# imdea-software/legosnark

Hardware: AMD Instinct MI355X
Metric: alt_bn128 G1 MSM point-scalar pairs/s at n=2^20 (higher is better)
Workload: dtype u32 limbs (254-bit Montgomery integers)

## Files before the change

legosnark_amd/csrc/msm.hip:

```cpp
#include <hip/hip_runtime.h>
#include <stdint.h>
#include <stdio.h>
#include <stdlib.h>
#include <string.h>
#include <algorithm>
#include <type_traits>
#include <vector>

#include "curves.h"
#include "fp29x2l.h"
#include "fs29.h"
#include "glv.h"
#include "msm.h"
#include "msm_plan.h"

namespace lsa {

unsigned msm_window_bits(size_t n) {
    unsigned lg = 0;
    while ((size_t(1) << (lg + 1)) <= n) lg++;
    int c = (int)lg - 4;
    if (c < 8) c = 8;
    if (c > 16) c = 16;
    return (unsigned)c;
// ... 375 lines not shown
    for (uint32_t x = threadIdx.x; x < (Bc + 1) / 2; x += blockDim.x) cnt2[x] = 0;
    __syncthreads();
    const uint32_t t = xcd_tile(blockIdx.x, gridDim.x);
    const size_t lo = (size_t)t * tile;
    for (uint32_t il = threadIdx.x; il < tile; il += blockDim.x) {
        const size_t i = lo + il;
        if (i >= n) break;
        const uint32_t seg = segment_of(segs, (uint32_t)i);
        wide_digits(scalars[i], pl, seg * B, [&](unsigned, int32_t sd) {
            if (sd != 0) {
                const uint32_t b = cm.bin((uint32_t)(sd < 0 ? -sd : sd) - 1);
                atomicAdd(&cnt2[b >> 1], 1u << ((b & 1) * 16));
            }
        });
    }
    __syncthreads();
    uint16_t *th = tile_hist + (size_t)t * pitch;
    const uint16_t *c16 = reinterpret_cast<const uint16_t *>(cnt2);
    for (uint32_t x = threadIdx.x; x < Bc; x += blockDim.x) th[x] = c16[x];
}

template <int REC>
__global__ __launch_bounds__(1024) void k_scatter_wide(const Fr *__restrict__ scalars, size_t n, SegList segs, WidePlan pl, uint32_t B,
                                                       uint32_t Bc, uint32_t pitch, uint32_t tile, const uint32_t *__restrict__ hist_c,
                                                       uint32_t *__restrict__ offs, const uint32_t *__restrict__ tile_base,
                                                       void *__restrict__ out, uint32_t win_stride) {
    extern __shared__ __attribute__((aligned(16))) uint32_t base[];
    __shared__ uint32_t wsum[16];
    const uint32_t t = xcd_tile(blockIdx.x, gridDim.x);
    const uint32_t *tb = tile_base + (size_t)t * pitch;
    {
        const uint32_t per = (Bc + 1023) / 1024, b0 = threadIdx.x * per;
        uint32_t sum = 0;
        for (uint32_t q = 0; q < per; q++) if (b0 + q < Bc) sum += hist_c[b0 + q];
        uint32_t incl = sum;
#pragma unroll
        for (int d = 1; d < 64; d <<= 1) {
            const uint32_t u = __shfl_up(incl, d, 64);
            if ((int)(threadIdx.x & 63) >= d) incl += u;
        }
        if ((threadIdx.x & 63) == 63) wsum[threadIdx.x >> 6] = incl;
        __syncthreads();
        uint32_t run = incl - sum;
        for (uint32_t w = 0; w < (threadIdx.x >> 6); w++) run += wsum[w];
        for (uint32_t q = 0; q < per; q++) {
            const uint32_t b = b0 + q;
            if (b < Bc) {
                if (blockIdx.x == 0) offs[b] = run;
                base[b] = run + tb[b];
                run += hist_c[b];
            }
        }
    }
    __syncthreads();
    const size_t lo = (size_t)t * tile;
    for (uint32_t il = threadIdx.x; il < tile; il += 1024) {
        const size_t i = lo + il;
        if (i >= n) break;
        const uint32_t seg = segment_of(segs, (uint32_t)i);
        const uint32_t local = (uint32_t)i - segs.off[seg];
        wide_digits(scalars[i], pl, seg * B, [&](unsigned k, int32_t sd) {
            if (sd != 0) {
                const uint32_t b = (uint32_t)(sd < 0 ? -sd : sd) - 1;
                const uint32_t ent = (local + k * win_stride) | (sd < 0 ? 0x80000000u : 0u);
                if (REC == 1) ((uint64_t *)out)[atomicAdd(&base[b >> 7], 1u)] = ((uint64_t)(b & 127u) << 32) | ent;
                else if (REC == 2) ((uint32_t *)out)[atomicAdd(&base[b >> 6], 1u)] = (ent & 0x81ffffffu) | ((b & 63u) << 25);
                else ((uint32_t *)out)[atomicAdd(&base[b], 1u)] = ent;
            }
        });
    }
}

__device__ __forceinline__ uint32_t lds_inc_rank(uint32_t *counters, uint32_t idx) {
    const uint32_t first = (uint32_t)__builtin_amdgcn_readfirstlane((int)idx);
    const uint64_t active = __ballot(1), same = __ballot(idx == first);
    if (same == active) {
        const uint32_t rank = __builtin_amdgcn_mbcnt_hi((uint32_t)(active >> 32), __builtin_amdgcn_mbcnt_lo((uint32_t)active, 0u));
        uint32_t base = 0;
        if (rank == 0) base = atomicAdd(&counters[first], (uint32_t)__popcll(active));
        return (uint32_t)__builtin_amdgcn_readfirstlane((int)base) + rank;
    }
    return atomicAdd(&counters[idx], 1u);
}
#define PART_TILE 2048u
#define PART_SEGS 768u
#define PART_STAGE 28672u
__global__ __launch_bounds__(1024) void k_partition(const Fr *__restrict__ scalars, size_t n, SegList segs, WidePlan pl, uint32_t B, uint32_t Bc,
                                                    CoarseMap cm, uint32_t pitch, const uint16_t *__restrict__ tile_hist,
                                                    const uint32_t *__restrict__ hist_c, uint32_t *__restrict__ offs_c,
                                                    const uint32_t *__restrict__ tile_base, uint32_t *__restrict__ recs) {
    __builtin_amdgcn_s_setprio(3);
    extern __shared__ __attribute__((aligned(16))) uint32_t stage[];
    __shared__ uint32_t lstart[PART_SEGS + 1], lcur[PART_SEGS], gdst[PART_SEGS], wtot[2][PART_SEGS / 64];
    const uint32_t t = xcd_tile(blockIdx.x, gridDim.x);
    const unsigned lane = threadIdx.x & 63, wv = threadIdx.x >> 6;
    {
        uint32_t gv = 0, lv = 0;
        if (threadIdx.x < Bc) { gv = hist_c[threadIdx.x]; lv = tile_hist[(size_t)t * pitch + threadIdx.x]; }
        uint32_t gi = gv, li = lv;
#pragma unroll
        for (int d = 1; d < 64; d <<= 1) {
            const uint32_t a = __shfl_up(gi, d, 64), b = __shfl_up(li, d, 64);
            if ((int)lane >= d) { gi += a; li += b; }
        }
        if (wv < PART_SEGS / 64 && lane == 63) { wtot[0][wv] = gi; wtot[1][wv] = li; }
        __syncthreads();
        if (threadIdx.x < Bc) {
            uint32_t gex = gi - gv, lex = li - lv;
            for (unsigned w = 0; w < wv; w++) { gex += wtot[0][w]; lex += wtot[1][w]; }
            lstart[threadIdx.x] = lex;
            lcur[threadIdx.x] = lex;
            gdst[threadIdx.x] = gex + tile_base[(size_t)t * pitch + threadIdx.x];
            if (blockIdx.x == 0) offs_c[threadIdx.x] = gex;
            if (threadIdx.x == Bc - 1) lstart[Bc] = lex + lv;
        }
    }
    __syncthreads();
    const size_t lo = (size_t)t * PART_TILE;
    const uint32_t fine_bits = cm.sh_hi;
    const uint32_t tlow = t & ((1u << (16 - fine_bits)) - 1);
    for (uint32_t j = 0; j < PART_TILE / 1024; j++) {
        const uint32_t il = threadIdx.x + j * 1024;
        const size_t i = lo + il;
        if (i >= n) break;
        const uint32_t seg = segment_of(segs, (uint32_t)i);
        wide_digits(scalars[i], pl, seg * B, [&](unsigned k, int32_t sd) {
            if (sd != 0) {
                const uint32_t b = (uint32_t)(sd < 0 ? -sd : sd) - 1;
                const uint32_t pos = atomicAdd(&lcur[cm.bin(b)], 1u);
                stage[pos] = (tlow << (16 + fine_bits)) | (cm.fine(b) << 16) | (k << 12) | (sd < 0 ? 0x800u : 0u) | il;
            }
        });
    }
    __syncthreads();
    for (uint32_t sg = threadIdx.x >> 5; sg < Bc; sg += 32) {
        const uint32_t a = lstart[sg], e = lstart[sg + 1], g = gdst[sg];
        for (uint32_t x = a + (lane & 31); x < e; x += 32) recs[g + (x - a)] = stage[x];
    }
}

__global__ __launch_bounds__(1024) void k_fine_sort_part(const uint32_t *__restrict__ recs, const uint32_t *__restrict__ offs_c,
                                                         const uint32_t *__restrict__ hist_c, const uint32_t *__restrict__ tile_base,
                                                         uint32_t pitch, uint32_t T, CoarseMap cm, SegList segs, uint32_t win_stride, uint32_t stage_cap,
                                                         uint32_t *__restrict__ entries, uint32_t *__restrict__ hist, uint32_t *__restrict__ offs) {
    __builtin_amdgcn_s_setprio(3);
    extern __shared__ __attribute__((aligned(16))) uint32_t sm[];
    __shared__ uint32_t wsum[16];
    const uint32_t sg = blockIdx.x, lo = offs_c[sg], ns = hist_c[sg];
    const uint32_t fine_bits = cm.sh_hi, FM = 1u << fine_bits, fmask = FM - 1, tbits = 16 - fine_bits;
    const uint32_t F = 1u << cm.bits(sg), bucket0 = cm.first(sg);
    uint32_t *cnt = sm, *cur = sm + FM, *col = sm + 2 * FM, *stage = col + T + 1;
    const unsigned lane = threadIdx.x & 63, wv = threadIdx.x >> 6;
    for (uint32_t x = threadIdx.x; x < F; x += 1024) cnt[x] = 0;
    for (uint32_t x = threadIdx.x; x < T; x += 1024) col[x] = tile_base[(size_t)x * pitch + sg];
    if (threadIdx.x == 0) col[T] = ns;
    auto scan_counters = [&]() {
        const uint32_t per = (F + 1023) >> 10, f0 = threadIdx.x * per;
        uint32_t sum = 0;
        for (uint32_t q = 0; q < per; q++) if (f0 + q < F) sum += cnt[f0 + q];
        uint32_t incl = sum;
#pragma unroll
        for (int d = 1; d < 64; d <<= 1) {
            const uint32_t u = __shfl_up(incl, d, 64);
            if ((int)lane >= d) incl += u;
        }
        if (lane == 63) wsum[wv] = incl;
        __syncthreads();
        uint32_t run = incl - sum;
        for (unsigned w = 0; w < wv; w++) run += wsum[w];
        for (uint32_t q = 0; q < per; q++) {
            if (f0 + q >= F) break;
            const uint32_t c = cnt[f0 + q];
            cur[f0 + q] = run;
            hist[(size_t)bucket0 + f0 + q] = c;
            offs[(size_t)bucket0 + f0 + q] = lo + run;
            run += c;
        }
    };
    auto entry_of = [&](uint32_t r, uint32_t p2) {
        uint32_t a = 0, e = (T + (1u << tbits) - 1) >> tbits;
        while (e - a > 1) {
            const uint32_t m = (a + e) >> 1;
            if (col[m << tbits] <= p2) a = m; else e = m;
        }
        const uint32_t i = ((a << tbits) | (r >> (16 + fine_bits))) * PART_TILE + (r & 0x7ffu);
        const uint32_t local = i - segs.off[segment_of(segs, i)];
        return (local + ((r >> 12) & 15u) * win_stride) | ((r & 0x800u) << 20);
    };
    if (ns <= stage_cap) {
        constexpr uint32_t NR = PART_STAGE / 1024;
        uint32_t r[NR];
#pragma unroll
        for (uint32_t u = 0; u < NR; u++) { const uint32_t p2 = threadIdx.x + u * 1024; r[u] = p2 < ns ? recs[lo + p2] : 0u; }
        __syncthreads();
        uint16_t rk[NR];
#pragma unroll
        for (uint32_t u = 0; u < NR; u++) {
            rk[u] = 0;
            if (threadIdx.x + u * 1024 < ns) rk[u] = (uint16_t)atomicAdd(&cnt[(r[u] >> 16) & fmask], 1u);
        }
        __syncthreads();
        scan_counters();
        __syncthreads();
#pragma unroll
        for (uint32_t u = 0; u < NR; u++) {
            const uint32_t p2 = threadIdx.x + u * 1024;
            if (p2 < ns) stage[cur[(r[u] >> 16) & fmask] + rk[u]] = entry_of(r[u], p2);
        }
        __syncthreads();
        for (uint32_t x = threadIdx.x; x < ns; x += 1024) entries[lo + x] = stage[x];
        return;
    }
    __syncthreads();
    constexpr uint32_t UNR = 8;
    for (uint32_t p0 = threadIdx.x; p0 < ns; p0 += 1024 * UNR) {
        uint32_t r[UNR];
#pragma unroll
        for (uint32_t u = 0; u < UNR; u++) { const uint32_t p2 = p0 + u * 1024; r[u] = p2 < ns ? recs[lo + p2] : 0u; }
#pragma unroll
        for (uint32_t u = 0; u < UNR; u++) if (p0 + u * 1024 < ns) (void)lds_inc_rank(cnt, (r[u] >> 16) & fmask);
    }
    __syncthreads();
    scan_counters();
    __syncthreads();
    for (uint32_t p0 = threadIdx.x; p0 < ns; p0 += 1024 * UNR) {
        uint32_t r[UNR];
#pragma unroll
        for (uint32_t u = 0; u < UNR; u++) { const uint32_t p2 = p0 + u * 1024; r[u] = p2 < ns ? recs[lo + p2] : 0u; }
#pragma unroll
        for (uint32_t u = 0; u < UNR; u++) {
            const uint32_t p2 = p0 + u * 1024;
            if (p2 >= ns) break;
            entries[lo + lds_inc_rank(cur, (r[u] >> 16) & fmask)] = entry_of(r[u], p2);
        }
    }
}

template <class Rec>
struct RecOps;
template <>
struct RecOps<uint64_t> {
    static constexpr uint32_t NF = 128;
    static __device__ __forceinline__ uint32_t fine(uint64_t r) { return (uint32_t)(r >> 32); }
    static __device__ __forceinline__ uint32_t entry(uint64_t r) { return (uint32_t)r; }
};
template <>
struct RecOps<uint32_t> {
    static constexpr uint32_t NF = 64;
    static __device__ __forceinline__ uint32_t fine(uint32_t r) { return (r >> 25) & 63u; }
    static __device__ __forceinline__ uint32_t entry(uint32_t r) { return r & 0x81ffffffu; }
};
template <class Rec>
__global__ __launch_bounds__(1024) void k_fine_sort(const Rec *__restrict__ recs, const uint32_t *__restrict__ offs_c,
                                                    const uint32_t *__restrict__ hist_c, uint32_t *__restrict__ entries,
                                                    uint32_t *__restrict__ hist, uint32_t *__restrict__ offs) {
    using O = RecOps<Rec>;
    constexpr uint32_t NF = O::NF;
    __shared__ uint32_t cnt[NF], cur[NF];
    const uint32_t bin = blockIdx.x, lo = offs_c[bin], n = hist_c[bin];
    if (threadIdx.x < NF) cnt[threadIdx.x] = 0;
    __syncthreads();
    for (uint32_t j = threadIdx.x; j < n; j += 1024) atomicAdd(&cnt[O::fine(recs[lo + j])], 1u);
    __syncthreads();
    if (threadIdx.x < 64) {
        constexpr uint32_t PER = NF / 64;
        uint32_t c[PER], tot = 0;
#pragma unroll
        for (uint32_t q = 0; q < PER; q++) { c[q] = cnt[PER * threadIdx.x + q]; tot += c[q]; }
        uint32_t incl = tot;
#pragma unroll
        for (int d = 1; d < 64; d <<= 1) {
            uint32_t t = __shfl_up(incl, d, 64);
            if ((int)threadIdx.x >= d) incl += t;
        }
        uint32_t ex = incl - tot;
#pragma unroll
        for (uint32_t q = 0; q < PER; q++) {
            cur[PER * threadIdx.x + q] = ex;
            hist[(size_t)bin * NF + PER * threadIdx.x + q] = c[q];
            offs[(size_t)bin * NF + PER * threadIdx.x + q] = lo + ex;
            ex += c[q];
        }
    }
    __syncthreads();
    for (uint32_t j = threadIdx.x; j < n; j += 1024) {
        const Rec r = recs[lo + j];
        const uint32_t pos = atomicAdd(&cur[O::fine(r)], 1u);
        entries[lo + pos] = O::entry(r);
    }
}

#define SIZE_BINS 1025
__device__ __forceinline__ uint32_t size_bin(uint32_t cnt, uint32_t bin_shift) { return ((cnt - 1) >> bin_shift) + 1; }
template <class C>
__global__ __launch_bounds__(256) void k_size_hist(const uint32_t *__restrict__ hist, uint32_t nb, uint32_t thr, uint32_t *__restrict__ bin_count,
                                                   uint32_t group_size, uint32_t bin_shift) {
    bin_count += (group_size ? (blockIdx.x * 2048u) / group_size : 0u) * SIZE_BINS;
    __shared__ uint32_t lcnt[SIZE_BINS];
    for (uint32_t t = threadIdx.x; t < SIZE_BINS; t += 256) lcnt[t] = 0;
    __syncthreads();
    const uint32_t base = blockIdx.x * 2048 + threadIdx.x;
#pragma unroll
    for (int j = 0; j < 8; j++) {
        uint32_t g = base + j * 256;
        if (g < nb) { uint32_t cnt = hist[g]; if (cnt > 0 && cnt <= thr) atomicAdd(&lcnt[size_bin(cnt, bin_shift)], 1u); }
    }
    __syncthreads();
    for (uint32_t t = threadIdx.x; t < SIZE_BINS; t += 256) if (lcnt[t]) atomicAdd(&bin_count[t], lcnt[t]);
}
__global__ __launch_bounds__(256) void k_size_scan(const uint32_t *__restrict__ bin_count, uint32_t *__restrict__ bin_start, uint32_t ngroups) {
    __shared__ uint32_t lds[4];
    uint32_t carry = 0;
    for (uint32_t gidx = 0; gidx < ngroups; gidx++) {
        const uint32_t *bc = bin_count + gidx * SIZE_BINS;
        uint32_t *bs = bin_start + gidx * SIZE_BINS;
        uint32_t v[4], s = 0;
#pragma unroll
        for (int j = 0; j < 4; j++) {
            int bin = (int)SIZE_BINS - 1 - (int)(threadIdx.x * 4 + j);
            v[j] = (bin >= 1) ? bc[bin] : 0;
            s += v[j];
        }
        uint32_t tot;
        uint32_t run = carry + block_exclusive_scan_256(s, lds, &tot);
#pragma unroll
        for (int j = 0; j < 4; j++) {
            int bin = (int)SIZE_BINS - 1 - (int)(threadIdx.x * 4 + j);
            if (bin >= 1) bs[bin] = run;
            run += v[j];
        }
        carry += tot;
    }
    if (threadIdx.x == 0) bin_start[0] = carry;
}
template <class C>
__global__ __launch_bounds__(256) void k_size_scatter(const uint32_t *__restrict__ hist, uint32_t nb, uint32_t thr, const uint32_t *__restrict__ bin_start,
                                                      uint32_t *__restrict__ bin_cursor, uint32_t *__restrict__ perm,
                                                      uint32_t *__restrict__ heavy_list, uint32_t *__restrict__ heavy_count,
                                                      typename C::Acc *__restrict__ buckets, uint32_t group_size, uint32_t bin_shift,
                                                      uint32_t split) {
    const uint32_t goff = (group_size ? (blockIdx.x * 2048u) / group_size : 0u) * SIZE_BINS;
    bin_start += goff;
    bin_cursor += goff;
    __shared__ uint32_t lcnt[SIZE_BINS];
    for (uint32_t t = threadIdx.x; t < SIZE_BINS; t += 256) lcnt[t] = 0;
    __syncthreads();
    const uint32_t base = blockIdx.x * 2048 + threadIdx.x;
    uint32_t cnt[8], rank[8];
#pragma unroll
    for (int j = 0; j < 8; j++) {
        uint32_t g = base + j * 256;
        cnt[j] = 0; rank[j] = 0;
        if (g < nb) {
            cnt[j] = hist[g];
            if (cnt[j] == 0) { for (uint32_t h = 0; h < split; h++) buckets[(size_t)g * split + h] = C::inf(); }
            else if (cnt[j] > thr) heavy_list[atomicAdd(heavy_count, 1u)] = g;
            else rank[j] = atomicAdd(&lcnt[size_bin(cnt[j], bin_shift)], 1u);
        }
    }
    __syncthreads();
    for (uint32_t t = threadIdx.x; t < SIZE_BINS; t += 256) {
        uint32_t c = lcnt[t];
        lcnt[t] = c ? atomicAdd(&bin_cursor[t], c) : 0;
    }
    __syncthreads();
#pragma unroll
    for (int j = 0; j < 8; j++) {
        uint32_t g = base + j * 256;
        if (g < nb && cnt[j] > 0 && cnt[j] <= thr) {
            const uint32_t bin = size_bin(cnt[j], bin_shift);
            perm[bin_start[bin] + lcnt[bin] + rank[j]] = g;
        }
    }
}

template <class C, uint32_t ACC_SPLIT>
__device__ __forceinline__ void accumulate_body(const typename C::Base *__restrict__ bases, const uint32_t *__restrict__ entries,
                                                const uint32_t *__restrict__ offs, const uint32_t *__restrict__ hist,
                                                const uint32_t *__restrict__ perm, const uint32_t *__restrict__ nperm,
                                                typename C::Acc *__restrict__ buckets) {
    uint32_t t = blockIdx.x * blockDim.x + threadIdx.x;
    if (t >= *nperm * ACC_SPLIT) return;
    const uint32_t g = perm[t / ACC_SPLIT], part = t % ACC_SPLIT;
    const uint32_t cnt = hist[g];
    const uint32_t *e = entries + offs[g];
    typename C::Acc acc = C::inf();
    if (part < cnt) {
        uint32_t v = e[part];
        typename C::Base cur = bases[v & 0x3fffffffu];
        for (uint32_t j = part; j < cnt; j += ACC_SPLIT) {
            uint32_t vn = v;
            typename C::Base nxt = cur;
            if (j + ACC_SPLIT < cnt) { vn = e[j + ACC_SPLIT]; nxt = bases[vn & 0x3fffffffu]; }
            acc = C::madd(acc, cur, (v >> 31) != 0, ((v >> 30) & 1) != 0);
            v = vn;
            cur = nxt;
        }
    }
    buckets[(size_t)g * ACC_SPLIT + part] = acc;
}
template <class C, uint32_t ACC_SPLIT>
__global__ __launch_bounds__(256) void k_accumulate(const typename C::Base *__restrict__ bases, const uint32_t *__restrict__ entries,
                                                    const uint32_t *__restrict__ offs, const uint32_t *__restrict__ hist,
                                                    const uint32_t *__restrict__ perm, const uint32_t *__restrict__ nperm,
                                                    typename C::Acc *__restrict__ buckets) {
    accumulate_body<C, ACC_SPLIT>(bases, entries, offs, hist, perm, nperm, buckets);
}
__global__ __launch_bounds__(256) __attribute__((amdgpu_waves_per_eu(2, 2))) void k_accumulate_g2_occ2(
    const CurveG2::Base *__restrict__ bases, const uint32_t *__restrict__ entries, const uint32_t *__restrict__ offs,
    const uint32_t *__restrict__ hist, const uint32_t *__restrict__ perm, const uint32_t *__restrict__ nperm, CurveG2::Acc *__restrict__ buckets) {
    accumulate_body<CurveG2, 1u>(bases, entries, offs, hist, perm, nperm, buckets);
}

__global__ __launch_bounds__(256) void k_accumulate_g2_pair(const AffPackedG2 *__restrict__ bases, const uint32_t *__restrict__ entries,
                                                            const uint32_t *__restrict__ offs, const uint32_t *__restrict__ hist,
                                                            const uint32_t *__restrict__ perm, const uint32_t *__restrict__ nperm,
                                                            XYZZ29x2 *__restrict__ buckets) {
    const uint32_t t = blockIdx.x * blockDim.x + threadIdx.x, pr = t >> 1, part = t & 1;
    if (pr >= *nperm) return;
    const uint32_t g = perm[pr];
    const uint32_t cnt = hist[g];
    const uint32_t *e = entries + offs[g];
    struct Half { uint32_t x[8], y[8]; };
    auto fetch = [&](uint32_t v) {
        const AffPackedG2 &b = bases[v & 0x3fffffffu];
        Half h;
#pragma unroll
        for (int i = 0; i < 8; i++) { h.x[i] = b.w[part][i]; h.y[i] = b.w[2 + part][i]; }
        return h;
    };
    XyzzE<F29h> acc = XyzzE<F29h>::inf();
    uint32_t v = e[0];
    Half cur = fetch(v);
    for (uint32_t j = 0; j < cnt; j++) {
        uint32_t vn = v;
        Half nxt = cur;
        if (j + 1 < cnt) { vn = e[j + 1]; nxt = fetch(vn); }
        AffE<F29h> q = {{F29::unpack256(cur.x)}, {F29::unpack256(cur.y)}};
        if (!q.is_inf()) {
            if (v >> 31) q.y = sub_k<1>(F29h::zero(), q.y);
            acc = g2_madd(acc, q);
        }
        v = vn;
        cur = nxt;
    }
    F29 *o = reinterpret_cast<F29 *>(&buckets[g]);
    o[part] = acc.X.v;
    o[2 + part] = acc.Y.v;
    o[4 + part] = acc.ZZ.v;
    o[6 + part] = acc.ZZZ.v;
}

template <class A>
__device__ __forceinline__ A shfl_down_acc(const A &p, unsigned delta) {
    A r;
// ... 663 lines not shown
    typename C::Base *tbl = (typename C::Base *)d_table;
    hipLaunchKernelGGL((k_shift_window<C>), dim3((unsigned)((n + 255) / 256)), dim3(256), 0, st, tbl + (size_t)(k - 1) * n, (Jac<F> *)d_tmp, n, grid.pos[k] - grid.pos[k - 1]);
    return prepare_bases<F>((const Jac<F> *)d_tmp, tbl + (size_t)k * n, n, st);
}
template int precompute_window_step<Fq>(void *, size_t, void *, unsigned, hipStream_t);
template int precompute_window_step<Fq2>(void *, size_t, void *, unsigned, hipStream_t);
template int precompute_windows<Fq>(void *, size_t, hipStream_t);
template int precompute_windows<Fq2>(void *, size_t, hipStream_t);

unsigned msm_field_mults_per_pair(size_t n, size_t table_n) {
    if (table_n && n >= table_use_min()) return wide_plan(table_n, n, 1).nwin * 10;
    return 16 * 10 + 8;
}

template <class F>
static int msm_pipeline(const void *d_bases_v, size_t first, const Fr *d_scalars, const SegList &segs, Jac<F> *d_out, hipStream_t st,
                        size_t table_stride, bool reuse_sort = false, bool blocking = false) {
    using C = typename CurveOf<F>::type;
    using A = typename C::Acc;
    const typename C::Base *d_bases = (const typename C::Base *)d_bases_v + first;
    const uint32_t nseg = segs.nseg;
    const size_t n = segs.off[nseg];
    if (n >= (size_t(1) << 27)) { set_error("msm: n too large (%zu)", n); return LSA_ERR_INVALID; }
    const bool wide = table_stride != 0 && (nseg > 1 || n >= table_use_min());
    if (nseg > 1 && !wide) { set_error("msm: segmented calls need bases with pre-shifted copies"); return LSA_ERR_INVALID; }
    WidePlan pl = {};
    if (wide) {
        pl = wide_plan(table_stride, n, nseg);
        if ((uint64_t)table_stride * table_copies(table_stride) >= (1u << 30)) { set_error("msm: base table too large for 30-bit entries"); return LSA_ERR_INVALID; }
    }
    const bool glv = C::GLV && !wide;
    const unsigned c = wide ? pl.c : msm_window_bits(glv ? 2 * n : n);
    const unsigned nwin = wide ? pl.nwin : (glv ? (128 + c - 1) / c : num_windows(c));
    const size_t nv = glv ? 2 * n : n;
    const uint32_t B = 1u << (c - 1);
    const uint32_t nb = wide ? nseg * B : nwin * B;
    if (wide && (uint64_t)nseg * B > (1u << 21)) { set_error("msm: %u segments of %u buckets exceed the bin space", nseg, B); return LSA_ERR_INVALID; }
    const bool fine = wide && nb > 32768;
    static const bool allow_rec32 = getenv("LSA_NO_REC32") == nullptr;
    const bool rec32 = fine && allow_rec32 && (uint64_t)table_stride * table_copies(table_stride) < (1u << 25) && (nb >> 6) <= 32768;
    static const bool allow_part = getenv("LSA_NO_PART") == nullptr;
    const bool part = fine && allow_part && nseg == 1 && nwin <= 13 && n <= ((size_t)1 << 25) && (nb & (nb - 1)) == 0 && nb >= (1u << 19);
    const uint32_t fine_bits = rec32 ? 6u : WIDE_FINE_BITS;
    CoarseMap cm = {0u, 0u, fine ? fine_bits : 0u, 0u};
    uint32_t Bc = !wide ? B : (fine ? nb >> fine_bits : nb);
    if (part) {
        bool narrower = false;
        for (unsigned k = 0; k < nwin; k++) narrower |= pl.width[k] < c;
        unsigned lg = 0;
        while ((1u << lg) < B) lg++;
        if (narrower) { cm.half = B >> 1; cm.sh_lo = lg - 1 - 9; cm.sh_hi = lg - 1 - 8; cm.nlo = 512; Bc = 768; }
        else { cm.half = 0; cm.sh_lo = cm.sh_hi = lg - 9; cm.nlo = 0; Bc = 512; }
    }
    const size_t ne = nv * nwin;
    const bool big = wide && B > 4096;
    static const uint32_t wide_split = getenv("LSA_WIDE_SPLIT") ? (uint32_t)atoi(getenv("LSA_WIDE_SPLIT")) : 1u;
    const uint32_t split = wide ? (wide_split == 2 ? 2u : 1u) : 2u;
    const uint32_t L = big ? std::max<uint32_t>(1, B / 65536) : (B > 4096 ? B / 4096 : 1);
    uint32_t logL = 0;
    while ((1u << logL) < L) logL++;
    const uint32_t T = B / L;
    const uint32_t wpw = big ? T : (T + 15) / 16;
    const uint32_t kw = wide ? nseg : nwin;
    const uint32_t avg_pop = (uint32_t)(ne / nb + 1);
    uint32_t pop_lo = avg_pop;
    if (wide && big) {
        unsigned nfull = 0;
        for (unsigned k = 0; k < nwin; k++) nfull += pl.width[k] == c;
        pop_lo = (uint32_t)(((uint64_t)n * (nfull + 2 * (nwin - nfull))) / B + 1);
    }
    const uint32_t heavy_threshold = (wide && !big) ? 4u : (wide ? std::max<uint32_t>(64, 2 * pop_lo + 32) : std::max<uint32_t>(64, 2 * avg_pop + 32));
    uint32_t bin_shift = 0;
    while (((heavy_threshold - 1) >> bin_shift) + 1 > SIZE_BINS - 1) bin_shift++;
    const uint32_t max_heavy = (uint32_t)std::min<size_t>(nb, ne / heavy_threshold + 1);
    const size_t max_chunks = ne / HEAVY_CHUNK + max_heavy + 1;

    size_t off = 0;
    auto carve = [&](size_t bytes) { size_t o = off; off = align_up(off + bytes, 256); return o; };
    size_t o_hist = carve((size_t)nb * 4 + 256);
    size_t o_offs = carve((size_t)nb * 4);
    const uint32_t nscan = wide ? Bc : nb;
    const uint32_t scan_blocks = (nscan + SCAN_PER_BLOCK - 1) / SCAN_PER_BLOCK;
    size_t o_bsum = carve((size_t)scan_blocks * 4);
    const uint32_t ngroups = 1;
    size_t o_bins = carve((size_t)3 * ngroups * SIZE_BINS * 4);
    size_t o_perm = carve((size_t)nb * 4);
    const uint32_t ntiles = (uint32_t)((nv + SORT_TILE - 1) / SORT_TILE);
    const uint32_t wtile = part ? PART_TILE : wide_tile(nwin, n);
    const uint32_t wtiles = (uint32_t)((n + wtile - 1) / wtile);
    const size_t rows = wide ? wtiles : (size_t)nwin * ntiles;
    size_t o_digits = carve(wide ? 0 : ne * 4);
    size_t o_rank = carve(wide ? 0 : ne * 2);
    const uint32_t pitch = wide ? Bc + 96 : Bc;
    size_t o_thist = carve(rows * pitch * 2);
    size_t o_tbase = carve(rows * pitch * 4);
    size_t o_entries = carve(ne * 4);
    size_t o_heavy = carve((size_t)max_heavy * 4);
    size_t o_choff = carve((size_t)(max_heavy + 2) * 4);
    size_t o_hpart = carve(max_chunks * sizeof(A));
    size_t o_recs = carve(fine ? ne * (part || rec32 ? 4 : 8) : 0);
    size_t o_chist = carve(fine ? (size_t)Bc * 4 : 0);
    size_t o_coffs = carve(fine ? (size_t)Bc * 4 : 0);
    if (g_ws.ensure(off) != 0) { set_error("msm: workspace allocation of %zu bytes failed", off); return LSA_ERR_NOMEM; }
    { int rcs = tail_slots_ready(); if (rcs) return rcs; }
    TailBuf &tb = g_tail[g_slot];
    TailBuf &prev = g_tail[(g_slot + tail_slots() - 1) % tail_slots()];
    hipStream_t tail = (g_overlap && !blocking) ? tb.stream : st;
    size_t toff = 0;
    auto tcarve = [&](size_t bytes) { size_t o = toff; toff = align_up(toff + bytes, 256); return o; };
    size_t o_buckets = tcarve((size_t)nb * split * sizeof(A));
    size_t o_wave = tcarve((size_t)kw * wpw * 2 * sizeof(A));
    size_t o_win = tcarve((size_t)kw * ((wpw + 15) / 16) * 2 * sizeof(A));
    size_t o_res = tcarve((size_t)nseg * sizeof(Jac<F>));
    for (auto &t : g_tail) {
        if (toff <= t.ws.cap || (blocking && &t != &tb)) continue;
        if (t.pending) HIPCHK(hipEventSynchronize(t.done));
        if (t.ws.ensure(toff) != 0) { set_error("msm: tail workspace allocation of %zu bytes failed", toff); return LSA_ERR_NOMEM; }
    }
    if (tb.pending) HIPCHK(hipStreamWaitEvent(st, tb.done, 0));
    tb.out = d_out;
    char *tws = (char *)tb.ws.ptr;
    char *ws = (char *)g_ws.ptr;
    uint32_t *hist = (uint32_t *)(ws + o_hist);
    uint32_t *heavy_count = hist + nb;
    uint32_t *offs = (uint32_t *)(ws + o_offs);
    uint32_t *bsum = (uint32_t *)(ws + o_bsum);
    uint32_t *bin_count = (uint32_t *)(ws + o_bins), *bin_start = bin_count + ngroups * SIZE_BINS, *bin_cursor = bin_start + ngroups * SIZE_BINS;
    uint32_t *perm = (uint32_t *)(ws + o_perm);
    int32_t *digits = (int32_t *)(ws + o_digits);
    uint16_t *rank = (uint16_t *)(ws + o_rank);
    uint16_t *tile_hist = (uint16_t *)(ws + o_thist);
    uint32_t *tile_base = (uint32_t *)(ws + o_tbase);
    uint32_t *entries = (uint32_t *)(ws + o_entries);
    A *buckets = (A *)(tws + o_buckets);
    uint32_t *heavy_list = (uint32_t *)(ws + o_heavy);
    uint32_t *chunk_off = (uint32_t *)(ws + o_choff);
    A *hpart = (A *)(ws + o_hpart);
    uint64_t *recs = (uint64_t *)(ws + o_recs);
    uint32_t *hist_c = fine ? (uint32_t *)(ws + o_chist) : hist;
    uint32_t *offs_c = fine ? (uint32_t *)(ws + o_coffs) : offs;
    A *wave_out = (A *)(tws + o_wave);
    A *window_sums = (A *)(tws + o_win);

    if (g_profile && !g_ev_ready) {
        for (auto &row : g_ev) for (auto &e : row) HIPCHK(hipEventCreate(&e));
        g_ev_ready = true;
    }
    int evi = 0;
    const int evslot = g_ev_calls % EV_POOL;
    auto mark = [&](hipStream_t s_) { if (g_profile) (void)hipEventRecord(g_ev[evslot][evi++], s_); };

    mark(st);
    { int rca = msm_func_attrs(); if (rca) return rca; }
    if (reuse_sort) {
        if (!wide) { set_error("msm: a shared sort needs bases with pre-shifted copies"); return LSA_ERR_INVALID; }
        mark(st); mark(st); mark(st);
    } else if (wide) {
        const uint32_t win_stride = (uint32_t)(table_stride * pl.copy_step);
        hipLaunchKernelGGL(k_hist_wide, dim3(wtiles), dim3(1024), (size_t)((Bc + 1) / 2) * 4, st, d_scalars, n, segs, pl, B, Bc, cm, pitch, wtile, tile_hist);
        mark(st);
        hipLaunchKernelGGL(k_tile_scan_rows, dim3((Bc + 31) / 32), dim3(1024), 0, st, tile_hist, Bc, wtiles, pitch, tile_base, hist_c, heavy_count, bin_count,
                           (uint32_t)(3 * ngroups * SIZE_BINS));
        mark(st);
        if (part) {
            hipLaunchKernelGGL(k_partition, dim3(wtiles), dim3(1024), (size_t)nwin * PART_TILE * 4, st, d_scalars, n, segs, pl, B, Bc, cm, pitch,
                               tile_hist, hist_c, offs_c, tile_base, (uint32_t *)recs);
            const uint32_t fixed_words = 2 * (1u << cm.sh_hi) + wtiles + 1, budget_words = 155648 / 4;
            const uint32_t stage_cap = fixed_words + PART_STAGE <= budget_words ? PART_STAGE : 0u;
            hipLaunchKernelGGL(k_fine_sort_part, dim3(Bc), dim3(1024), (size_t)(fixed_words + stage_cap) * 4, st, (const uint32_t *)recs, offs_c, hist_c,
                               tile_base, pitch, wtiles, cm, segs, win_stride, stage_cap, entries, hist, offs);
        } else if (rec32) {
            hipLaunchKernelGGL(k_scatter_wide<2>, dim3(wtiles), dim3(1024), (size_t)Bc * 4, st, d_scalars, n, segs, pl, B, Bc, pitch, wtile, hist_c, offs_c, tile_base, (void *)recs, win_stride);
            hipLaunchKernelGGL(k_fine_sort<uint32_t>, dim3(Bc), dim3(1024), 0, st, (const uint32_t *)recs, offs_c, hist_c, entries, hist, offs);
        } else if (fine) {
            hipLaunchKernelGGL(k_scatter_wide<1>, dim3(wtiles), dim3(1024), (size_t)Bc * 4, st, d_scalars, n, segs, pl, B, Bc, pitch, wtile, hist_c, offs_c, tile_base, (void *)recs, win_stride);
            hipLaunchKernelGGL(k_fine_sort<uint64_t>, dim3(Bc), dim3(1024), 0, st, (const uint64_t *)recs, offs_c, hist_c, entries, hist, offs);
        } else {
            hipLaunchKernelGGL(k_scatter_wide<0>, dim3(wtiles), dim3(1024), (size_t)Bc * 4, st, d_scalars, n, segs, pl, B, Bc, pitch, wtile, hist_c, offs_c, tile_base, (void *)entries, win_stride);
        }
        mark(st);
    } else {
        hipLaunchKernelGGL((k_digits<C::GLV>), dim3((unsigned)((n + 255) / 256)), dim3(256), 0, st, d_scalars, n, c, nwin, digits);
        hipLaunchKernelGGL(k_rank, dim3(ntiles, nwin), dim3(1024), (size_t)B * 2, st, digits, nv, B, ntiles, rank, tile_hist, 0u);
        hipLaunchKernelGGL(k_tile_scan, dim3((nb + 255) / 256), dim3(256), 0, st, tile_hist, B, ntiles, nb, tile_base, hist);
        mark(st);
        hipLaunchKernelGGL(k_scan_sums, dim3(scan_blocks), dim3(256), 0, st, hist, nb, bsum);
        hipLaunchKernelGGL(k_scan_blocks, dim3(1), dim3(256), 0, st, bsum, scan_blocks);
        hipLaunchKernelGGL(k_scan_final, dim3(scan_blocks), dim3(256), 0, st, hist, bsum, nb, offs);
        mark(st);
        hipLaunchKernelGGL(k_scatter, dim3(ntiles, nwin), dim3(1024), (size_t)B * 4, st, digits, rank, offs, tile_base, nv, n, B, ntiles, entries, 0u);
        mark(st);
    }
    if (!wide || reuse_sort) {
        HIPCHK(hipMemsetAsync(heavy_count, 0, 4, st));
        HIPCHK(hipMemsetAsync(bin_count, 0, (size_t)3 * ngroups * SIZE_BINS * 4, st));
    }
    {
        const unsigned sb = (nb + 2047) / 2048;
        const uint32_t gsz = 0u;
        hipLaunchKernelGGL((k_size_hist<C>), dim3(sb), dim3(256), 0, st, hist, nb, heavy_threshold, bin_count, gsz, bin_shift);
        hipLaunchKernelGGL(k_size_scan, dim3(1), dim3(256), 0, st, bin_count, bin_start, ngroups);
        hipLaunchKernelGGL((k_size_scatter<C>), dim3(sb), dim3(256), 0, st, hist, nb, heavy_threshold, bin_start, bin_cursor, perm, heavy_list, heavy_count, buckets, gsz, bin_shift, split);
    }
    mark(st);
    static const bool g2_pair = getenv("LSA_G2_PAIR") && getenv("LSA_G2_PAIR")[0] == '1';
    if constexpr (std::is_same<C, CurveG2>::value) {
        if (split == 1 && g2_pair) {
            hipLaunchKernelGGL(k_accumulate_g2_pair, dim3((nb * 2 + 255) / 256), dim3(256), 0, st, d_bases, entries, offs, hist, perm, bin_start, buckets);
            goto acc_done;
        }
        if (split == 1) {
            hipLaunchKernelGGL(k_accumulate_g2_occ2, dim3((nb + 255) / 256), dim3(256), 0, st, d_bases, entries, offs, hist, perm, bin_start, buckets);
            goto acc_done;
        }
    }
    if (split == 1)
        hipLaunchKernelGGL((k_accumulate<C, 1u>), dim3((nb + 255) / 256), dim3(256), 0, st, d_bases, entries, offs, hist, perm, bin_start, buckets);
    else
        hipLaunchKernelGGL((k_accumulate<C, 2u>), dim3((nb * 2 + 255) / 256), dim3(256), 0, st, d_bases, entries, offs, hist, perm, bin_start, buckets);
acc_done:
    hipLaunchKernelGGL(k_heavy_plan, dim3(1), dim3(256), 0, st, hist, heavy_list, heavy_count, chunk_off);
    hipLaunchKernelGGL((k_accumulate_heavy<C>), dim3(4096), dim3(64), 0, st, d_bases, entries, offs, hist,
                       heavy_list, heavy_count, chunk_off, hpart);
    hipLaunchKernelGGL((k_heavy_finish<C>), dim3(256), dim3(64), 0, st, heavy_list, heavy_count, chunk_off, hpart, buckets, split);
    mark(st);
    if (tail != st) HIPCHK(hipEventRecord(tb.front_done, st));
    const bool profile = g_profile;
    hipEvent_t ev6 = profile ? g_ev[evslot][6] : nullptr, ev7 = profile ? g_ev[evslot][7] : nullptr;
    const size_t res_off = o_res;
    {
        if (tail != st) HIPCHK(hipStreamWaitEvent(tail, tb.front_done, 0));
        if (big)
            hipLaunchKernelGGL((k_reduce1_lane<C>), dim3(kw * ((T + 63) / 64)), dim3(64), 0, tail, buckets, B, L, split, wave_out);
        else
            hipLaunchKernelGGL((k_reduce1<C>), dim3(kw * wpw), dim3(64), 0, tail, buckets, B, L, logL, wpw, split, wave_out);
        A *lvl_in = wave_out, *lvl_out = window_sums;
        uint32_t m = wpw, lm = big ? logL : logL + 4;
        static const bool allow_bits = getenv("LSA_NO_REDUCE_BITS") == nullptr;
        const bool bits_tail = allow_bits && blocking && big && kw == 1 && nseg == 1 && m >= 4096 && (m / 16) <= 8192;
        bool converted = false;
        Jac<F> *res = tail != st ? (Jac<F> *)(tws + res_off) : d_out;
        static const bool allow_lane_l1 = getenv("LSA_NO_LANE_L1") == nullptr;
        static const bool g2_lane_l1 = getenv("LSA_G2_LANE_L1") != nullptr && getenv("LSA_G2_LANE_L1")[0] == '1';
        bool lane_l1 = allow_lane_l1 && (std::is_same<C, CurveG1>::value || g2_lane_l1) && !blocking && !reuse_sort && big && kw == 1 && nseg == 1 && m >= 16384 &&
                       tail != st && prev.pending && prev.unjoined && &prev != &tb;
        do {
            const uint32_t m_out = (m + 15) / 16;
            if (lane_l1) {
                hipLaunchKernelGGL((k_reduce2_lane<C>), dim3((m_out + 63) / 64), dim3(64), 0, tail, lvl_in, m, m_out, lm, lvl_out);
                lane_l1 = false;
            } else
            hipLaunchKernelGGL((k_reduce2<C>), dim3(kw * m_out), dim3(64), 0, tail, lvl_in, m, m_out, lm, lvl_out);
            std::swap(lvl_in, lvl_out);
            m = m_out;
            lm += 4;
            if (bits_tail && m > 1) {
                uint32_t nbits = 0;
                while ((1u << nbits) < m) nbits++;
                const uint32_t G = (m + 511) / 512;
                A *part = lvl_out;
                A *weighted = part + (size_t)(nbits + 1) * G;
                hipLaunchKernelGGL((k_reduce_bits_a<C>), dim3(nbits + 1, G), dim3(512), 0, tail, lvl_in, m, nbits, G, part);
                hipLaunchKernelGGL((k_reduce_bits_b<C>), dim3(nbits + 1), dim3(64), 0, tail, part, nbits, G, lm, weighted);
                if (profile) (void)hipEventRecord(ev6, tail);
                hipLaunchKernelGGL((k_reduce_bits_c<C>), dim3(1), dim3(64), 0, tail, weighted, nbits + 1, res);
                converted = true;
                break;
            }
        } while (m > 1);
        if (!converted && profile) (void)hipEventRecord(ev6, tail);
        if (converted) {
        } else if (wide && nseg > 1) {
            if constexpr (std::is_same<C, CurveG1>::value) hipLaunchKernelGGL(k_emit_g1, dim3(nseg), dim3(64), 0, tail, lvl_in, res);
            else hipLaunchKernelGGL(k_emit_g2, dim3(nseg), dim3(64), 0, tail, lvl_in, res);
        } else if constexpr (std::is_same<C, CurveG1>::value) {
            hipLaunchKernelGGL(k_fold_quad, dim3(1), dim3(64), 0, tail, lvl_in, kw, c, res);
        } else {
            hipLaunchKernelGGL(k_fold_quad_g2, dim3(1), dim3(64), 0, tail, lvl_in, kw, c, res);
        }
        if (tail != st) {
            if (prev.pending && &prev != &tb) HIPCHK(hipStreamWaitEvent(tail, prev.done, 0));
            for (int i = 0; i < NTAIL; i++) {
                TailBuf &o = g_tail[i];
                if (&o != &tb && &o != &prev && o.pending && o.out == (const void *)d_out) HIPCHK(hipStreamWaitEvent(tail, o.done, 0));
            }
            hipLaunchKernelGGL(k_publish, dim3(1), dim3(256), 0, tail, (const uint32_t *)res, (uint32_t *)d_out, (unsigned)(nseg * sizeof(Jac<F>) / 4));
        }
        if (profile) (void)hipEventRecord(ev7, tail);
        HIPCHK(hipEventRecord(tb.done, tail));
    }
    tb.pending = true;
    tb.unjoined = (tail != st);
    if (!blocking) g_slot = (g_slot + 1) % tail_slots();
    HIPCHK(hipGetLastError());
    if (g_profile) g_ev_calls++;
    return LSA_OK;
}

template <class F>
int msm_device(const void *d_bases_v, size_t first, const Fr *d_scalars, size_t n, Jac<F> *d_out, hipStream_t st, size_t table_stride, bool blocking) {
    if (n == 0) {
        int jr = msm_join(st);
// ... 60 lines not shown
```

Measured before the change: 769.1 million.

## Fuse bucket-size histogram into fine sort and fold size scan into scatter

The bucket-size histogram is now computed inside k_fine_sort_part from the LDS counters it already holds, so the separate k_size_hist pass over hist is skipped on the partition path. The single-block k_size_scan launch is removed; each k_size_scatter block recomputes the exclusive scan of bin counts in LDS, and the total is written to nperm for the accumulate kernels. This removes two small launches and one global read of hist. In exchange, the fine sort uses extra LDS (which can shrink the staging capacity), does global atomics into bin_count, and every scatter block repeats the scan.

New measurement: 775.2 million, median of 6. Within noise of the previous version (+0.8%).

```diff
diff --git a/legosnark_amd/csrc/msm.hip b/legosnark_amd/csrc/msm.hip
--- a/legosnark_amd/csrc/msm.hip
+++ b/legosnark_amd/csrc/msm.hip
@@ -481,6 +481,8 @@
     }
     return atomicAdd(&counters[idx], 1u);
 }
+#define SIZE_BINS 1025
+__device__ __forceinline__ uint32_t size_bin(uint32_t cnt, uint32_t bin_shift) { return ((cnt - 1) >> bin_shift) + 1; }
 #define PART_TILE 2048u
 #define PART_SEGS 768u
 #define PART_STAGE 28672u
@@ -541,6 +543,7 @@
 __global__ __launch_bounds__(1024) void k_fine_sort_part(const uint32_t *__restrict__ recs, const uint32_t *__restrict__ offs_c,
                                                          const uint32_t *__restrict__ hist_c, const uint32_t *__restrict__ tile_base,
                                                          uint32_t pitch, uint32_t T, CoarseMap cm, SegList segs, uint32_t win_stride, uint32_t stage_cap,
+                                                         uint32_t thr, uint32_t bin_shift, uint32_t *__restrict__ bin_count,
                                                          uint32_t *__restrict__ entries, uint32_t *__restrict__ hist, uint32_t *__restrict__ offs) {
     __builtin_amdgcn_s_setprio(3);
     extern __shared__ __attribute__((aligned(16))) uint32_t sm[];
@@ -548,9 +551,10 @@
     const uint32_t sg = blockIdx.x, lo = offs_c[sg], ns = hist_c[sg];
     const uint32_t fine_bits = cm.sh_hi, FM = 1u << fine_bits, fmask = FM - 1, tbits = 16 - fine_bits;
     const uint32_t F = 1u << cm.bits(sg), bucket0 = cm.first(sg);
-    uint32_t *cnt = sm, *cur = sm + FM, *col = sm + 2 * FM, *stage = col + T + 1;
+    uint32_t *cnt = sm, *cur = sm + FM, *sizes = sm + 2 * FM, *col = sizes + SIZE_BINS, *stage = col + T + 1;
     const unsigned lane = threadIdx.x & 63, wv = threadIdx.x >> 6;
     for (uint32_t x = threadIdx.x; x < F; x += 1024) cnt[x] = 0;
+    for (uint32_t x = threadIdx.x; x < SIZE_BINS; x += 1024) sizes[x] = 0;
     for (uint32_t x = threadIdx.x; x < T; x += 1024) col[x] = tile_base[(size_t)x * pitch + sg];
     if (threadIdx.x == 0) col[T] = ns;
     auto scan_counters = [&]() {
@@ -576,6 +580,14 @@
             run += c;
         }
     };
+    auto count_sizes = [&]() {
+        for (uint32_t f = threadIdx.x; f < F; f += 1024) {
+            const uint32_t c = cnt[f];
+            if (c > 0 && c <= thr) atomicAdd(&sizes[size_bin(c, bin_shift)], 1u);
+        }
+        __syncthreads();
+        for (uint32_t x = threadIdx.x; x < SIZE_BINS; x += 1024) if (sizes[x]) atomicAdd(&bin_count[x], sizes[x]);
+    };
     auto entry_of = [&](uint32_t r, uint32_t p2) {
         uint32_t a = 0, e = (T + (1u << tbits) - 1) >> tbits;
         while (e - a > 1) {
@@ -608,6 +620,7 @@
         }
         __syncthreads();
         for (uint32_t x = threadIdx.x; x < ns; x += 1024) entries[lo + x] = stage[x];
+        count_sizes();
         return;
     }
     __syncthreads();
@@ -633,6 +646,7 @@
             entries[lo + lds_inc_rank(cur, (r[u] >> 16) & fmask)] = entry_of(r[u], p2);
         }
     }
+    count_sizes();
 }
 
 template <class Rec>
@@ -689,12 +703,9 @@
     }
 }
 
-#define SIZE_BINS 1025
-__device__ __forceinline__ uint32_t size_bin(uint32_t cnt, uint32_t bin_shift) { return ((cnt - 1) >> bin_shift) + 1; }
 template <class C>
 __global__ __launch_bounds__(256) void k_size_hist(const uint32_t *__restrict__ hist, uint32_t nb, uint32_t thr, uint32_t *__restrict__ bin_count,
-                                                   uint32_t group_size, uint32_t bin_shift) {
-    bin_count += (group_size ? (blockIdx.x * 2048u) / group_size : 0u) * SIZE_BINS;
+                                                   uint32_t bin_shift) {
     __shared__ uint32_t lcnt[SIZE_BINS];
     for (uint32_t t = threadIdx.x; t < SIZE_BINS; t += 256) lcnt[t] = 0;
     __syncthreads();
@@ -707,43 +718,31 @@
     __syncthreads();
     for (uint32_t t = threadIdx.x; t < SIZE_BINS; t += 256) if (lcnt[t]) atomicAdd(&bin_count[t], lcnt[t]);
 }
-__global__ __launch_bounds__(256) void k_size_scan(const uint32_t *__restrict__ bin_count, uint32_t *__restrict__ bin_start, uint32_t ngroups) {
-    __shared__ uint32_t lds[4];
-    uint32_t carry = 0;
-    for (uint32_t gidx = 0; gidx < ngroups; gidx++) {
-        const uint32_t *bc = bin_count + gidx * SIZE_BINS;
-        uint32_t *bs = bin_start + gidx * SIZE_BINS;
+template <class C>
+__global__ __launch_bounds__(256) void k_size_scatter(const uint32_t *__restrict__ hist, uint32_t nb, uint32_t thr, const uint32_t *__restrict__ bin_count,
+                                                      uint32_t *__restrict__ bin_cursor, uint32_t *__restrict__ nperm, uint32_t *__restrict__ perm,
+                                                      uint32_t *__restrict__ heavy_list, uint32_t *__restrict__ heavy_count,
+                                                      typename C::Acc *__restrict__ buckets, uint32_t bin_shift, uint32_t split) {
+    __shared__ uint32_t lcnt[SIZE_BINS], lstart[SIZE_BINS], lds[4];
+    for (uint32_t t = threadIdx.x; t < SIZE_BINS; t += 256) lcnt[t] = 0;
+    {
         uint32_t v[4], s = 0;
 #pragma unroll
         for (int j = 0; j < 4; j++) {
-            int bin = (int)SIZE_BINS - 1 - (int)(threadIdx.x * 4 + j);
-            v[j] = (bin >= 1) ? bc[bin] : 0;
+            const int bin = (int)SIZE_BINS - 1 - (int)(threadIdx.x * 4 + j);
+            v[j] = bin >= 1 ? bin_count[bin] : 0;
             s += v[j];
         }
         uint32_t tot;
-        uint32_t run = carry + block_exclusive_scan_256(s, lds, &tot);
+        uint32_t run = block_exclusive_scan_256(s, lds, &tot);
 #pragma unroll
         for (int j = 0; j < 4; j++) {
-            int bin = (int)SIZE_BINS - 1 - (int)(threadIdx.x * 4 + j);
-            if (bin >= 1) bs[bin] = run;
+            const int bin = (int)SIZE_BINS - 1 - (int)(threadIdx.x * 4 + j);
+            if (bin >= 1) lstart[bin] = run;
             run += v[j];
         }
-        carry += tot;
-    }
-    if (threadIdx.x == 0) bin_start[0] = carry;
-}
-template <class C>
-__global__ __launch_bounds__(256) void k_size_scatter(const uint32_t *__restrict__ hist, uint32_t nb, uint32_t thr, const uint32_t *__restrict__ bin_start,
-                                                      uint32_t *__restrict__ bin_cursor, uint32_t *__restrict__ perm,
-                                                      uint32_t *__restrict__ heavy_list, uint32_t *__restrict__ heavy_count,
-                                                      typename C::Acc *__restrict__ buckets, uint32_t group_size, uint32_t bin_shift,
-                                                      uint32_t split) {
-    const uint32_t goff = (group_size ? (blockIdx.x * 2048u) / group_size : 0u) * SIZE_BINS;
-    bin_start += goff;
-    bin_cursor += goff;
-    __shared__ uint32_t lcnt[SIZE_BINS];
-    for (uint32_t t = threadIdx.x; t < SIZE_BINS; t += 256) lcnt[t] = 0;
-    __syncthreads();
+        if (blockIdx.x == 0 && threadIdx.x == 0) *nperm = tot;
+    }
     const uint32_t base = blockIdx.x * 2048 + threadIdx.x;
     uint32_t cnt[8], rank[8];
 #pragma unroll
@@ -760,16 +759,13 @@
     __syncthreads();
     for (uint32_t t = threadIdx.x; t < SIZE_BINS; t += 256) {
         uint32_t c = lcnt[t];
-        lcnt[t] = c ? atomicAdd(&bin_cursor[t], c) : 0;
+        lcnt[t] = c ? lstart[t] + atomicAdd(&bin_cursor[t], c) : 0;
     }
     __syncthreads();
 #pragma unroll
     for (int j = 0; j < 8; j++) {
         uint32_t g = base + j * 256;
-        if (g < nb && cnt[j] > 0 && cnt[j] <= thr) {
-            const uint32_t bin = size_bin(cnt[j], bin_shift);
-            perm[bin_start[bin] + lcnt[bin] + rank[j]] = g;
-        }
+        if (g < nb && cnt[j] > 0 && cnt[j] <= thr) perm[lcnt[size_bin(cnt[j], bin_shift)] + rank[j]] = g;
     }
 }
 
@@ -1599,8 +1595,8 @@
     const uint32_t nscan = wide ? Bc : nb;
     const uint32_t scan_blocks = (nscan + SCAN_PER_BLOCK - 1) / SCAN_PER_BLOCK;
     size_t o_bsum = carve((size_t)scan_blocks * 4);
-    const uint32_t ngroups = 1;
-    size_t o_bins = carve((size_t)3 * ngroups * SIZE_BINS * 4);
+    const uint32_t order_words = 2 * SIZE_BINS;
+    size_t o_bins = carve((size_t)(order_words + 1) * 4);
     size_t o_perm = carve((size_t)nb * 4);
     const uint32_t ntiles = (uint32_t)((nv + SORT_TILE - 1) / SORT_TILE);
     const uint32_t wtile = part ? PART_TILE : wide_tile(nwin, n);
@@ -1642,7 +1638,7 @@
     uint32_t *heavy_count = hist + nb;
     uint32_t *offs = (uint32_t *)(ws + o_offs);
     uint32_t *bsum = (uint32_t *)(ws + o_bsum);
-    uint32_t *bin_count = (uint32_t *)(ws + o_bins), *bin_start = bin_count + ngroups * SIZE_BINS, *bin_cursor = bin_start + ngroups * SIZE_BINS;
+    uint32_t *bin_count = (uint32_t *)(ws + o_bins), *bin_cursor = bin_count + SIZE_BINS, *nperm = bin_count + order_words;
     uint32_t *perm = (uint32_t *)(ws + o_perm);
     int32_t *digits = (int32_t *)(ws + o_digits);
     uint16_t *rank = (uint16_t *)(ws + o_rank);
@@ -1677,15 +1673,15 @@
         hipLaunchKernelGGL(k_hist_wide, dim3(wtiles), dim3(1024), (size_t)((Bc + 1) / 2) * 4, st, d_scalars, n, segs, pl, B, Bc, cm, pitch, wtile, tile_hist);
         mark(st);
         hipLaunchKernelGGL(k_tile_scan_rows, dim3((Bc + 31) / 32), dim3(1024), 0, st, tile_hist, Bc, wtiles, pitch, tile_base, hist_c, heavy_count, bin_count,
-                           (uint32_t)(3 * ngroups * SIZE_BINS));
+                           order_words);
         mark(st);
         if (part) {
             hipLaunchKernelGGL(k_partition, dim3(wtiles), dim3(1024), (size_t)nwin * PART_TILE * 4, st, d_scalars, n, segs, pl, B, Bc, cm, pitch,
                                tile_hist, hist_c, offs_c, tile_base, (uint32_t *)recs);
-            const uint32_t fixed_words = 2 * (1u << cm.sh_hi) + wtiles + 1, budget_words = 155648 / 4;
+            const uint32_t fixed_words = 2 * (1u << cm.sh_hi) + SIZE_BINS + wtiles + 1, budget_words = 155648 / 4;
             const uint32_t stage_cap = fixed_words + PART_STAGE <= budget_words ? PART_STAGE : 0u;
             hipLaunchKernelGGL(k_fine_sort_part, dim3(Bc), dim3(1024), (size_t)(fixed_words + stage_cap) * 4, st, (const uint32_t *)recs, offs_c, hist_c,
-                               tile_base, pitch, wtiles, cm, segs, win_stride, stage_cap, entries, hist, offs);
+                               tile_base, pitch, wtiles, cm, segs, win_stride, stage_cap, heavy_threshold, bin_shift, bin_count, entries, hist, offs);
         } else if (rec32) {
             hipLaunchKernelGGL(k_scatter_wide<2>, dim3(wtiles), dim3(1024), (size_t)Bc * 4, st, d_scalars, n, segs, pl, B, Bc, pitch, wtile, hist_c, offs_c, tile_base, (void *)recs, win_stride);
             hipLaunchKernelGGL(k_fine_sort<uint32_t>, dim3(Bc), dim3(1024), 0, st, (const uint32_t *)recs, offs_c, hist_c, entries, hist, offs);
@@ -1710,31 +1706,30 @@
     }
     if (!wide || reuse_sort) {
         HIPCHK(hipMemsetAsync(heavy_count, 0, 4, st));
-        HIPCHK(hipMemsetAsync(bin_count, 0, (size_t)3 * ngroups * SIZE_BINS * 4, st));
+        HIPCHK(hipMemsetAsync(bin_count, 0, (size_t)order_words * 4, st));
     }
     {
         const unsigned sb = (nb + 2047) / 2048;
-        const uint32_t gsz = 0u;
-        hipLaunchKernelGGL((k_size_hist<C>), dim3(sb), dim3(256), 0, st, hist, nb, heavy_threshold, bin_count, gsz, bin_shift);
-        hipLaunchKernelGGL(k_size_scan, dim3(1), dim3(256), 0, st, bin_count, bin_start, ngroups);
-        hipLaunchKernelGGL((k_size_scatter<C>), dim3(sb), dim3(256), 0, st, hist, nb, heavy_threshold, bin_start, bin_cursor, perm, heavy_list, heavy_count, buckets, gsz, bin_shift, split);
+        if (!part || reuse_sort)
+            hipLaunchKernelGGL((k_size_hist<C>), dim3(sb), dim3(256), 0, st, hist, nb, heavy_threshold, bin_count, bin_shift);
+        hipLaunchKernelGGL((k_size_scatter<C>), dim3(sb), dim3(256), 0, st, hist, nb, heavy_threshold, bin_count, bin_cursor, nperm, perm, heavy_list, heavy_count, buckets, bin_shift, split);
     }
     mark(st);
     static const bool g2_pair = getenv("LSA_G2_PAIR") && getenv("LSA_G2_PAIR")[0] == '1';
     if constexpr (std::is_same<C, CurveG2>::value) {
         if (split == 1 && g2_pair) {
-            hipLaunchKernelGGL(k_accumulate_g2_pair, dim3((nb * 2 + 255) / 256), dim3(256), 0, st, d_bases, entries, offs, hist, perm, bin_start, buckets);
+            hipLaunchKernelGGL(k_accumulate_g2_pair, dim3((nb * 2 + 255) / 256), dim3(256), 0, st, d_bases, entries, offs, hist, perm, nperm, buckets);
             goto acc_done;
         }
         if (split == 1) {
-            hipLaunchKernelGGL(k_accumulate_g2_occ2, dim3((nb + 255) / 256), dim3(256), 0, st, d_bases, entries, offs, hist, perm, bin_start, buckets);
+            hipLaunchKernelGGL(k_accumulate_g2_occ2, dim3((nb + 255) / 256), dim3(256), 0, st, d_bases, entries, offs, hist, perm, nperm, buckets);
             goto acc_done;
         }
     }
     if (split == 1)
-        hipLaunchKernelGGL((k_accumulate<C, 1u>), dim3((nb + 255) / 256), dim3(256), 0, st, d_bases, entries, offs, hist, perm, bin_start, buckets);
+        hipLaunchKernelGGL((k_accumulate<C, 1u>), dim3((nb + 255) / 256), dim3(256), 0, st, d_bases, entries, offs, hist, perm, nperm, buckets);
     else
-        hipLaunchKernelGGL((k_accumulate<C, 2u>), dim3((nb * 2 + 255) / 256), dim3(256), 0, st, d_bases, entries, offs, hist, perm, bin_start, buckets);
+        hipLaunchKernelGGL((k_accumulate<C, 2u>), dim3((nb * 2 + 255) / 256), dim3(256), 0, st, d_bases, entries, offs, hist, perm, nperm, buckets);
 acc_done:
     hipLaunchKernelGGL(k_heavy_plan, dim3(1), dim3(256), 0, st, hist, heavy_list, heavy_count, chunk_off);
     hipLaunchKernelGGL((k_accumulate_heavy<C>), dim3(4096), dim3(64), 0, st, d_bases, entries, offs, hist,
```
